# tychedelia/josefine

Hardware: NVIDIA H100
Metric: Raft-group ticks/sec @ 64Ki groups x 5 replicas (higher is better)
Workload: dtype u64

## Files before the change

josefine_b200/csrc/sym_fold.cuh:

```cuda
#pragma once
#include "raft_device.cuh"

namespace jr {
#ifdef JR_DEVICE_CODE

struct SymMail {
  uint32_t hb, hb_commit;
  uint32_t ae, ae_nb, ae_id[JR_MAX_AE_BLOCKS];
  uint32_t mk;
  uint32_t hbr, hbr_commit, hbr_has;
  uint32_t ar, ar_head;
};

constexpr uint32_t SYM_ROWS = 8;
#ifndef JR_SYM_LANES
#define JR_SYM_LANES 128
#endif
constexpr uint32_t SYM_LANES = JR_SYM_LANES;
constexpr uint32_t SYM_ENC_L = 5, SYM_ENC_F = 3;
constexpr uint32_t SYM_SMEM_UNITS = 2 * SYM_ROWS + SYM_ENC_L + SYM_ENC_F;
constexpr uint32_t SYM2_GROUPS = 64;
constexpr uint32_t SYM2_UNITS = SYM_SMEM_UNITS + 2 * 2 + 2 * 1;
constexpr uint32_t SYM2_ABORT = 1u << 8, SYM2_IDS = 1u << 9, SYM2_MODE = 1u << 10;

template <int R, bool SPLIT = false>
struct SymGroup {
  static constexpr uint32_t STRIDE = SPLIT ? SYM2_GROUPS : SYM_LANES;
  const Dev& d;
  const uint32_t g;
  const size_t plane;
  uint32_t L;
  uint32_t F0;
  uint64_t term, hbtime, now;
  uint32_t head, commit, idgen, maxkey, ckey, ph_self, mode_self, ph_f, mode_f;
  uint32_t fhead, fcommit, fmaxkey, fckey;
  uint32_t n_hb;
  uint64_t last_hb;
  uint32_t tbase;
  uint32_t flo;
  uint4* rows;
  uint4* enc;
  uint32_t lcnt, fcnt;
  uint32_t n_app;
  bool abort;
  bool share;

  __device__ __forceinline__ SymGroup(const Dev& dv, uint32_t g_) : d(dv), g(g_), plane((size_t)R * dv.Gp) {}
  __device__ __forceinline__ size_t rg(uint32_t r) const { return (size_t)r * d.Gp + g; }
  __device__ __forceinline__ size_t row(uint32_t r, uint32_t bid) const { return (size_t)(bid & d.capm) * plane + rg(r); }
  __device__ __forceinline__ bool in_window(uint32_t bid) const { return bid - tbase < d.cap; }
  __device__ __forceinline__ uint4& slot(uint32_t r, uint32_t bid) const { return rows[((r == L ? 0u : SYM_ROWS) + (bid % SYM_ROWS)) * STRIDE]; }
  __device__ __forceinline__ void cache_put(uint32_t r, uint32_t bid, uint32_t nx, uint64_t tk) const {
    slot(r, bid) = make_uint4(bid, nx, (uint32_t)tk, (uint32_t)(tk >> 32));
  }
  __device__ __forceinline__ void fetch(uint32_t r, uint32_t bid, uint32_t& next, uint64_t& tok) {
    if (!in_window(bid)) { next = ABSENT; tok = 0; return; }
    const uint4 e = slot(r, bid);
    if (e.x == bid) { next = e.y; tok = (uint64_t)e.z | ((uint64_t)e.w << 32); return; }
    next = __ldcg(d.cnext + row(r, bid));
    tok = __ldcg(d.ctok + row(r, bid));
    if (!SPLIT) cache_put(r, bid, next, tok);
  }
  __device__ __forceinline__ void fetch_sent(uint32_t bid, uint32_t mk_sent, uint32_t n_app, uint32_t& next, uint64_t& tok) {
    if (!SPLIT) { fetch(L, bid, next, tok); return; }
    if (!in_window(bid)) { next = ABSENT; tok = 0; return; }
    if (bid + SYM_ROWS > mk_sent + n_app) {
      const uint4 e = slot(L, bid);
      if (e.x == bid) { next = e.y; tok = (uint64_t)e.z | ((uint64_t)e.w << 32); return; }
    }
    next = __ldcg(d.cnext + row(L, bid));
    tok = __ldcg(d.ctok + row(L, bid));
  }
  __device__ __forceinline__ void cache_clear(uint32_t first = 0, uint32_t n = 2 * SYM_ROWS) const {
#pragma unroll
    for (uint32_t k = 0; k < 2 * SYM_ROWS; ++k)
      if (k >= first && k < first + n) rows[k * STRIDE] = make_uint4(ABSENT, ABSENT, 0u, 0u);
  }
  __device__ __forceinline__ void cache_fill(uint32_t r, uint32_t top) const {
    uint32_t nx[SYM_ROWS];
    uint64_t tk[SYM_ROWS];
#pragma unroll
    for (uint32_t j = 0; j < SYM_ROWS; ++j)
      if (j <= top && in_window(top - j)) {
        nx[j] = d.cnext[row(r, top - j)];
        tk[j] = d.ctok[row(r, top - j)];
      }
#pragma unroll
    for (uint32_t j = 0; j < SYM_ROWS; ++j)
      if (j <= top && in_window(top - j)) cache_put(r, top - j, nx[j], tk[j]);
  }
  __device__ __forceinline__ bool has(uint32_t r, uint32_t bid) {
    uint32_t n; uint64_t t;
    fetch(r, bid, n, t);
    return n != ABSENT;
  }
  __device__ __forceinline__ void fetch_f(uint32_t bid, uint32_t& next, uint64_t& tok) {
    if (in_window(bid) && bid < flo) { abort = true; next = ABSENT; tok = 0; return; }
    fetch(F0, bid, next, tok);
  }
  __device__ __forceinline__ bool has_f(uint32_t bid) {
    uint32_t n; uint64_t t;
    fetch_f(bid, n, t);
    return n != ABSENT;
  }

  __device__ __forceinline__ uint4& eq(uint32_t k) const { return enc[k * STRIDE]; }
  __device__ __forceinline__ FsmOut leader_out() const { return FsmOut{d.fs + rg(L), plane, d.F, g, L}; }
  __device__ __forceinline__ FsmOut followers_out() const {
    return FsmOut{d.fs + rg(F0), plane, d.F, g, F0, ((1u << R) - 1u) & ~(1u << L)};
  }
  __device__ __forceinline__ void enc_init_leader(uint2 leader_fc) const {
    eq(0) = make_uint4(leader_fc.x, leader_fc.y, leader_fc.y, 0u);
#pragma unroll
    for (uint32_t k = 1; k < SYM_ENC_L; ++k) eq(k) = make_uint4(0u, 0u, 0u, 0u);
  }
  __device__ __forceinline__ void enc_init_followers() const {
#pragma unroll
    for (uint32_t k = SYM_ENC_L; k < SYM_ENC_L + SYM_ENC_F; ++k) eq(k) = make_uint4(0u, 0u, 0u, 0u);
  }
  template <bool NOTIFY>
  __device__ __forceinline__ void emit_leader(uint32_t bid, uint32_t nxa, uint64_t tok) {
    if (!(d.flags & JR_F_CAPTURE_FSM)) return;
    if (lcnt >= d.Fr) { abort = true; return; }
    FsmEnc e;
    const uint4 q0 = eq(0);
    e.nrec = q0.x; e.seq = q0.y + lcnt; e.wseq = q0.z; e.pb2 = q0.w;
    ++lcnt;
    const bool window = NOTIFY || e.seq + 1u - e.wseq == FS_PATTERN_BITS;
    uint4 q1 = make_uint4(0u, 0u, 0u, 0u);
    if (window) q1 = eq(1);
    e.pb0 = (uint64_t)q1.x | ((uint64_t)q1.y << 32);
    e.pb1 = (uint64_t)q1.z | ((uint64_t)q1.w << 32);
    const uint4 qr = eq(NOTIFY ? 4 : 2), qs = eq(3);
    FsmRun& run = NOTIFY ? e.rn : e.ra;
    run.next_id = qr.x; run.count = qr.y;
    run.last = (uint64_t)qr.z | ((uint64_t)qr.w << 32);
    run.stride = NOTIFY ? ((uint64_t)qs.z | ((uint64_t)qs.w << 32)) : ((uint64_t)qs.x | ((uint64_t)qs.y << 32));
    fsm_enc_push<NOTIFY>(e, leader_out(), bid, nxa, tok);
    if (e.nrec != q0.x || e.wseq != q0.z || e.pb2 != q0.w) eq(0) = make_uint4(e.nrec, q0.y, e.wseq, e.pb2);
    if (window) eq(1) = make_uint4((uint32_t)e.pb0, (uint32_t)(e.pb0 >> 32), (uint32_t)e.pb1, (uint32_t)(e.pb1 >> 32));
    eq(NOTIFY ? 4 : 2) = make_uint4(run.next_id, run.count, (uint32_t)run.last, (uint32_t)(run.last >> 32));
    uint2* st = reinterpret_cast<uint2*>(&eq(3)) + (NOTIFY ? 1 : 0);
    *st = make_uint2((uint32_t)run.stride, (uint32_t)(run.stride >> 32));
  }
  __device__ __forceinline__ uint2 leader_end() {
    FsmEnc e;
    const uint4 q0 = eq(0), q1 = eq(1), q2 = eq(2), q3 = eq(3), q4 = eq(4);
    e.nrec = q0.x; e.seq = q0.y + lcnt; e.wseq = q0.z; e.pb2 = q0.w;
    e.pb0 = (uint64_t)q1.x | ((uint64_t)q1.y << 32);
    e.pb1 = (uint64_t)q1.z | ((uint64_t)q1.w << 32);
    e.ra = FsmRun{q2.x, q2.y, (uint64_t)q2.z | ((uint64_t)q2.w << 32), (uint64_t)q3.x | ((uint64_t)q3.y << 32)};
    e.rn = FsmRun{q4.x, q4.y, (uint64_t)q4.z | ((uint64_t)q4.w << 32), (uint64_t)q3.z | ((uint64_t)q3.w << 32)};
    return fsm_enc_end(e, leader_out());
  }
  __device__ __forceinline__ void emit_followers(uint32_t bid, uint32_t next, uint64_t tok) {
    if (!(d.flags & JR_F_CAPTURE_FSM)) return;
    if (fcnt >= d.Fr) { abort = true; return; }
    if (share) {
      FsmEnc e;
      const uint4 q0 = eq(SYM_ENC_L), q1 = eq(SYM_ENC_L + 1);
      const uint2 q2 = *reinterpret_cast<const uint2*>(&eq(SYM_ENC_L + 2));
      e.nrec = q0.x; e.seq = q0.y + fcnt; e.wseq = q0.z; e.pb2 = 0;
      e.pb0 = e.pb1 = 0;
      e.ra = FsmRun{q1.x, q1.y, (uint64_t)q1.z | ((uint64_t)q1.w << 32), (uint64_t)q2.x | ((uint64_t)q2.y << 32)};
      fsm_enc_push<false>(e, followers_out(), bid, next, tok);
      if (e.nrec != q0.x || e.wseq != q0.z) eq(SYM_ENC_L) = make_uint4(e.nrec, q0.y, e.wseq, 0u);
      eq(SYM_ENC_L + 1) = make_uint4(e.ra.next_id, e.ra.count, (uint32_t)e.ra.last, (uint32_t)(e.ra.last >> 32));
      *reinterpret_cast<uint2*>(&eq(SYM_ENC_L + 2)) = make_uint2((uint32_t)e.ra.stride, (uint32_t)(e.ra.stride >> 32));
    } else {
      const uint4 e = make_uint4(bid, next, (uint32_t)tok, (uint32_t)(tok >> 32));
#pragma unroll
      for (int r = 0; r < R; ++r)
        if ((uint32_t)r != L) d.fr[(size_t)fcnt * plane + rg(r)] = e;
    }
    ++fcnt;
  }
  __device__ __forceinline__ uint2 followers_end() {
    FsmEnc e;
    const uint4 q0 = eq(SYM_ENC_L), q1 = eq(SYM_ENC_L + 1), q2 = eq(SYM_ENC_L + 2);
    e.nrec = q0.x; e.seq = q0.y + fcnt; e.wseq = q0.z; e.pb2 = 0;
    e.pb0 = e.pb1 = 0;
    e.ra = FsmRun{q1.x, q1.y, (uint64_t)q1.z | ((uint64_t)q1.w << 32), (uint64_t)q2.x | ((uint64_t)q2.y << 32)};
    e.rn = FsmRun{0, 0, 0, 0};
    return fsm_enc_end(e, followers_out());
  }

  __device__ __forceinline__ uint32_t committed_index(uint32_t v_new, uint32_t n_new, uint32_t v_old) const {
    uint32_t v[R];
    v[0] = ph_self;
#pragma unroll
    for (int i = 1; i < R; ++i) v[i] = (uint32_t)i <= n_new ? v_new : v_old;
#pragma unroll
    for (int i = 0; i < R; ++i)
#pragma unroll
      for (int j = 0; j + 1 < R - i; ++j) {
        const uint32_t a = v[j], b = v[j + 1];
        v[j] = max(a, b);
        v[j + 1] = min(a, b);
      }
    return v[R / 2];
  }
  __device__ __forceinline__ void leader_commit(uint32_t v_new, uint32_t n_new, uint32_t v_old) {
    const uint32_t above = (ph_self > commit ? 1u : 0u) + (v_new > commit ? n_new : 0u) + (v_old > commit ? (uint32_t)(R - 1) - n_new : 0u);
    if (above < (uint32_t)(R / 2 + 1)) return;
    const uint32_t q = committed_index(v_new, n_new, v_old);
    if (q <= commit) return;
    if (!has(L, q)) { abort = true; return; }
    const uint32_t prev = commit;
    ckey = 1;
    commit = q;
    bool first = true;
    for (uint32_t b = max(prev, tbase); b <= q; ++b) {
      uint32_t nx; uint64_t tk;
      fetch(L, b, nx, tk);
      if (nx == ABSENT) continue;
      if (first) { first = false; continue; }
      emit_leader<false>(b, nx, tk);
    }
  }
  __device__ __forceinline__ void client_request(uint64_t tok) {
    const uint32_t bid = idgen++;
    if (!(bid > head) || !in_window(bid)) { abort = true; return; }
    d.cnext[row(L, bid)] = head;
    d.ctok[row(L, bid)] = tok;
    cache_put(L, bid, head, tok);
    if (bid > maxkey) maxkey = bid;
    head = bid;
    emit_leader<true>(bid, FSR_CLIENT, tok);
    mode_self = ph_self < head ? 1u : 0u;
    if (ph_self < head) ph_self = head;
    leader_commit(ph_f, R - 1, ph_f);
  }

  __device__ __forceinline__ void leader_tick(const SymMail& in, SymMail& out, uint64_t dense_tok, uint32_t n_synth,
                                              uint64_t step_index) {
    if (in.hbr && !in.hbr_has && in.hbr_commit > 0) { abort = true; return; }
    if (in.ar) {
      const uint32_t old = ph_f, v = in.ar_head;
      const bool inc = old < v;
      const uint32_t nw = inc ? v : old;
      for (uint32_t j = 1; j <= (uint32_t)(R - 1) && !abort; ++j) leader_commit(nw, j, old);
      ph_f = nw;
      mode_f = inc ? 1u : 0u;
      if (abort) return;
    }
    if (dense_tok) client_request(dense_tok);
    for (uint32_t i = 0; i < n_synth && !abort; ++i) client_request(synth_token(step_index, i, d.goff + g));
    if (abort) return;
    const uint64_t el = now >= hbtime ? now - hbtime : 0;
    if (el > (uint64_t)d.hb) {
      out.hb = 1;
      out.hb_commit = commit;
      hbtime = now;
    }
    out.ae = 1;
    out.mk = maxkey;
    if (!SPLIT) replicate(ph_f, mode_f, maxkey, out);
  }
  __device__ __forceinline__ void replicate(uint32_t phf, uint32_t modef, uint32_t mk, SymMail& out) {
    const uint32_t take = modef ? JR_MAX_AE_BLOCKS : 1u;
    uint32_t bid = max(phf, tbase), pulled = 0, nb = 0;
    while (pulled < 1 + take) {
      uint32_t nx = ABSENT; uint64_t tk = 0;
      while (bid <= mk) {
        fetch(L, bid, nx, tk);
        if (nx != ABSENT) break;
        ++bid;
      }
      if (bid > mk) break;
      if (pulled >= 1) out.ae_id[nb++] = bid;
      ++pulled;
      ++bid;
    }
    out.ae_nb = nb;
  }

  __device__ __forceinline__ void follower_heartbeat(const SymMail& in, SymMail& out) {
    ++n_hb;
    last_hb = now;
    const uint32_t c = in.hb_commit;
    const bool hasc = has_f(c);
    if (hasc && c > fcommit) {
      const uint32_t prev = fcommit;
      fckey = 1;
      fcommit = c;
      for (uint32_t b = max(prev, tbase); b < c; ++b) {
        uint32_t nx; uint64_t tk;
        fetch_f(b, nx, tk);
        if (nx != ABSENT) emit_followers(b, nx, tk);
      }
    }
    out.hbr = 1;
    out.hbr_commit = fcommit;
    out.hbr_has = hasc ? 1u : 0u;
  }
  __device__ __forceinline__ void follower_extend(uint32_t bid, uint32_t nx, uint64_t tk) {
    if (nx == ABSENT || !has_f(nx) || !in_window(bid)) { abort = true; return; }
#pragma unroll
    for (int r = 0; r < R; ++r)
      if ((uint32_t)r != L) {
        d.cnext[row(r, bid)] = nx;
        d.ctok[row(r, bid)] = tk;
      }
    cache_put(F0, bid, nx, tk);
    if (bid > fmaxkey) fmaxkey = bid;
    fhead = bid;
  }
  __device__ __forceinline__ void follower_tick(const SymMail& in, SymMail& out) {
    if (in.hb) follower_heartbeat(in, out);
    if (in.ae) {
      for (uint32_t k = 0; k < in.ae_nb && !abort; ++k) {
        const uint32_t bid = in.ae_id[k];
        uint32_t nx; uint64_t tk;
        fetch_sent(bid, in.mk, n_app, nx, tk);
        follower_extend(bid, nx, tk);
      }
      if (abort) return;
      if (in.ae_nb) {
        out.ar = 1;
        out.ar_head = fhead;
      }
    }
  }
  __device__ __forceinline__ void follower_tick_view(const SymMail& in, uint32_t phf, uint32_t modef, uint32_t mk, SymMail& out) {
    if (in.hb) follower_heartbeat(in, out);
    if (!in.ae || abort) return;
    const uint32_t take = modef ? JR_MAX_AE_BLOCKS : 1u;
    uint32_t bid = max(phf, tbase), pulled = 0, nb = 0;
    while (pulled < 1 + take) {
      uint32_t nx = ABSENT; uint64_t tk = 0;
      while (bid <= mk) {
        fetch_sent(bid, mk, n_app, nx, tk);
        if (nx != ABSENT) break;
        ++bid;
      }
      if (bid > mk) break;
      if (pulled >= 1) {
        follower_extend(bid, nx, tk);
        if (abort) return;
        ++nb;
      }
      ++pulled;
      ++bid;
    }
    if (nb) {
      out.ar = 1;
      out.ar_head = fhead;
    }
  }
};

template <int R, bool SPLIT>
__device__ __forceinline__ bool sym_enter(SymGroup<R, SPLIT>& s, SymMail& m, const StepParams& p, int prv) {
  const Dev& d = s.d;
  if (s.g >= d.G) return false;
  uint32_t L = R, nlead = 0;
  uint4 p2[R];
#pragma unroll
  for (int r = 0; r < R; ++r) {
    p2[r] = d.p2[s.rg(r)];
    const uint32_t meta = p2[r].w;
    if (((meta >> 8) & 255u) || ((meta >> 27) & 1u)) return false;
    if ((meta & 255u) == JR_ROLE_LEADER) { L = r; ++nlead; }
    else if ((meta & 255u) != JR_ROLE_FOLLOWER) return false;
    if ((meta >> 24) & 7u) return false;
  }
  if (nlead != 1) return false;
  s.L = L;
  s.F0 = L == 0 ? 1u : 0u;
  const uint4 l0 = d.p0[s.rg(L)];
  s.term = (uint64_t)l0.x | ((uint64_t)l0.y << 32);
  s.tbase = d.tb[s.g];
  uint4 pl = p2[0], pf = p2[0];
  const uint32_t f0i = L == 0 ? 1u : 0u;
#pragma unroll
  for (int r = 0; r < R; ++r) {
    if ((uint32_t)r == L) pl = p2[r];
    if ((uint32_t)r == f0i) pf = p2[r];
  }
  s.head = pl.x; s.commit = pl.y; s.idgen = pl.z;
  s.ckey = (pl.w >> 28) & 1u;
  s.maxkey = d.mk[s.rg(L)];
  if (!(s.idgen > s.head)) return false;
  const uint4 l3 = d.p3[s.rg(L)];
  s.hbtime = (uint64_t)l3.x | ((uint64_t)l3.y << 32);
  const uint32_t f0 = s.F0;
  s.fhead = pf.x; s.fcommit = pf.y; s.fckey = (pf.w >> 28) & 1u;
  s.fmaxkey = d.mk[s.rg(f0)];
  const uint64_t hbgap = ((uint64_t)d.hb / p.dt + 1) * p.dt;
#pragma unroll
  for (int r = 0; r < R; ++r) {
    if ((uint32_t)r == L) continue;
    const uint4 a = d.p0[s.rg(r)];
    if (((uint64_t)a.x | ((uint64_t)a.y << 32)) != s.term || a.z != L + 1 || a.w != L + 1) return false;
    if (p2[r].x != s.fhead || p2[r].y != s.fcommit || ((p2[r].w >> 28) & 1u) != s.fckey) return false;
    if (d.mk[s.rg(r)] != s.fmaxkey) return false;
  }
  if ((uint64_t)d.emin <= hbgap || s.hbtime > p.now) return false;
  uint32_t ph[R];
#pragma unroll
  for (int q = 0; q < (R + 3) / 4; ++q) {
    const uint4 v = d.pr[(size_t)q * s.plane + s.rg(L)];
    if (q * 4 + 0 < R) ph[q * 4 + 0] = v.x;
    if (q * 4 + 1 < R) ph[q * 4 + 1] = v.y;
    if (q * 4 + 2 < R) ph[q * 4 + 2] = v.z;
    if (q * 4 + 3 < R) ph[q * 4 + 3] = v.w;
  }
  const uint32_t prmask = (pl.w >> 16) & 255u;
  s.ph_self = 0; s.ph_f = 0;
#pragma unroll
  for (int r = 0; r < R; ++r) {
    if ((uint32_t)r == L) s.ph_self = ph[r];
    if ((uint32_t)r == f0) s.ph_f = ph[r];
  }
  s.mode_self = (prmask >> L) & 1u;
  s.mode_f = (prmask >> f0) & 1u;
#pragma unroll
  for (int r = 0; r < R; ++r)
    if ((uint32_t)r != L && (ph[r] != s.ph_f || ((prmask >> r) & 1u) != s.mode_f)) return false;
  constexpr uint32_t SYM_WINDOW = 16;
  const uint32_t top = min(s.maxkey, s.fmaxkey);
  const uint32_t lo_min = max(top > SYM_WINDOW - 1u ? top - (SYM_WINDOW - 1u) : 0u, s.tbase);
  if (top < s.tbase || s.ph_f < lo_min || s.fcommit < lo_min || s.commit < lo_min || s.fhead < lo_min || s.fmaxkey > s.maxkey) return false;
  const uint32_t lo = min(min(s.ph_f, s.fcommit), min(s.commit, s.fhead));
  s.flo = lo;
  const uint64_t grow = (uint64_t)p.n_ticks * (1u + p.n_synth) + 2u;
  if ((uint64_t)s.maxkey + grow >= (uint64_t)s.tbase + d.cap || (uint64_t)s.maxkey + grow >= FS_NOTIFY_BIT) return false;
  {
    constexpr uint32_t B = 4;
    bool same = true;
    for (uint32_t b0 = lo; b0 <= s.fmaxkey && same; b0 += B) {
      uint32_t n0[B];
      unsigned long long t0[B];
#pragma unroll
      for (uint32_t j = 0; j < B; ++j) {
        const uint32_t b = min(b0 + j, s.fmaxkey);
        n0[j] = d.cnext[s.row(f0, b)];
        t0[j] = d.ctok[s.row(f0, b)];
      }
#pragma unroll
      for (int r = 0; r < R; ++r) {
        if ((uint32_t)r == L || (uint32_t)r == f0) continue;
#pragma unroll
        for (uint32_t j = 0; j < B; ++j) {
          const uint32_t b = min(b0 + j, s.fmaxkey);
          const uint32_t n = d.cnext[s.row(r, b)];
          const unsigned long long t = d.ctok[s.row(r, b)];
          same = same && n == n0[j] && (n0[j] == ABSENT || t == t0[j]);
        }
      }
    }
    if (!same) return false;
  }
  m = SymMail{};
  if (p.phases & PH_DRAIN) {
  {
    const uint32_t cnt = d.oc[prv][s.rg(L)];
    uint32_t u = 0;
    auto unit = [&](uint32_t k) { return d.ob[prv][((size_t)k * R + L) * d.Gp + s.g]; };
    if (cnt > (uint32_t)(1 + JR_MAX_AE_BLOCKS + R)) return false;
    if (u < cnt) {
      const uint4 h = unit(u);
      if ((h.x & 15u) == JR_CMD_HEARTBEAT) {
        if ((h.x >> 16) != TO_PEERS || ((uint64_t)h.y | ((uint64_t)h.z << 32)) != s.term) return false;
        m.hb = 1; m.hb_commit = h.w;
        ++u;
      }
    }
    if (u < cnt) {
      uint32_t first = 0;
      for (int r = 0; r < R; ++r) {
        if ((uint32_t)r == L) continue;
        if (u >= cnt) return false;
        const uint4 h = unit(u);
        if ((h.x & 15u) != JR_CMD_APPEND_ENTRIES || (h.x >> 16) != (uint32_t)r + 1u ||
            ((uint64_t)h.y | ((uint64_t)h.z << 32)) != s.term) return false;
        const uint32_t nb = (h.x >> 8) & 255u, ref = (h.x >> 4) & 1u;
        if (!m.ae) {
          if (ref || nb > JR_MAX_AE_BLOCKS || h.w != u + 1 || u + 1 + nb > cnt) return false;
          m.ae = 1; m.ae_nb = nb; first = u + 1;
          for (uint32_t k = 0; k < nb; ++k) {
            const uint4 bu = unit(first + k);
            uint32_t nx; uint64_t tk;
            s.fetch(L, bu.x, nx, tk);
            if (nx != bu.y || tk != ((uint64_t)bu.z | ((uint64_t)bu.w << 32))) return false;
            m.ae_id[k] = bu.x;
          }
          u += 1 + nb;
        } else {
          if (!ref || nb != m.ae_nb || h.w != first) return false;
          ++u;
        }
      }
    }
    if (u != cnt) return false;
  }
  {
    const uint32_t cnt = d.oc[prv][s.rg(f0)];
    if (cnt > 2) return false;
    uint4 want[2] = {make_uint4(0, 0, 0, 0), make_uint4(0, 0, 0, 0)};
    for (uint32_t u = 0; u < cnt; ++u) want[u] = d.ob[prv][((size_t)u * R + f0) * d.Gp + s.g];
#pragma unroll
    for (int r = 0; r < R; ++r) {
      if ((uint32_t)r == L || (uint32_t)r == f0) continue;
      if (d.oc[prv][s.rg(r)] != cnt) return false;
      for (uint32_t u = 0; u < cnt; ++u) {
        const uint4 v = d.ob[prv][((size_t)u * R + r) * d.Gp + s.g];
        if (v.x != want[u].x || v.y != want[u].y || v.z != want[u].z || v.w != want[u].w) return false;
      }
    }
    uint32_t u = 0;
    if (u < cnt && (want[u].x & 15u) == JR_CMD_HEARTBEAT_RESPONSE) {
      if ((want[u].x >> 16) != L + 1) return false;
      m.hbr = 1; m.hbr_has = (want[u].x >> 4) & 1u; m.hbr_commit = want[u].w;
      ++u;
    }
    if (u < cnt && (want[u].x & 15u) == JR_CMD_APPEND_RESPONSE) {
      if ((want[u].x >> 16) != L + 1 || ((uint64_t)want[u].y | ((uint64_t)want[u].z << 32)) != s.term) return false;
      m.ar = 1; m.ar_head = want[u].w;
      ++u;
    }
    if (u != cnt) return false;
  }
  }
  uint64_t t_arr = 0;
  if (!m.hb) {
    const uint64_t due = s.hbtime + (uint64_t)d.hb + 1;
    t_arr = (due > p.now ? (due - p.now + p.dt - 1) / p.dt : 0) + 1;
  }
  const uint64_t checked = t_arr < p.n_ticks ? t_arr : p.n_ticks;
  if (checked) {
    const uint64_t t_last = p.now + (checked - 1) * p.dt;
#pragma unroll
    for (int r = 0; r < R; ++r) {
      if ((uint32_t)r == L) continue;
      const uint4 b = d.p1[s.rg(r)];
      const uint64_t etime = (uint64_t)b.x | ((uint64_t)b.y << 32);
      if (t_last >= etime && t_last - etime > (uint64_t)b.z) return false;
    }
  }
  return true;
}

template <int R, bool SPLIT>
__device__ __forceinline__ void sym_leave_leader(SymGroup<R, SPLIT>& s, const SymMail& last, int cur_last) {
  const Dev& d = s.d;
  const uint32_t L = s.L;
  {
    const size_t i = s.rg(L);
    uint32_t prmask = 0;
#pragma unroll
    for (int r = 0; r < R; ++r) prmask |= (((uint32_t)r == L ? s.mode_self : s.mode_f) & 1u) << r;
    const uint32_t keep = d.p2[i].w & ~((255u << 16) | (1u << 28));
    d.p2[i] = make_uint4(s.head, s.commit, s.idgen, keep | (prmask << 16) | (s.ckey << 28));
    d.p3[i] = make_uint4((uint32_t)s.hbtime, (uint32_t)(s.hbtime >> 32), 0u, 0u);
#pragma unroll
    for (int q = 0; q < (R + 3) / 4; ++q) {
      uint32_t v[4] = {0, 0, 0, 0};
#pragma unroll
      for (int k = 0; k < 4; ++k)
        if (q * 4 + k < R) v[k] = (uint32_t)(q * 4 + k) == L ? s.ph_self : s.ph_f;
      d.pr[(size_t)q * s.plane + i] = make_uint4(v[0], v[1], v[2], v[3]);
    }
    d.mk[i] = s.maxkey;
    uint32_t u = 0;
    auto put = [&](uint32_t k, uint4 v) { d.ob[cur_last][((size_t)k * R + L) * d.Gp + s.g] = v; };
    if (last.hb) put(u++, make_uint4(unit_hdr(JR_CMD_HEARTBEAT, 0, 0, TO_PEERS), (uint32_t)s.term, (uint32_t)(s.term >> 32), last.hb_commit));
    if (last.ae) {
      uint32_t first = 0;
      bool have = false;
#pragma unroll
      for (int r = 0; r < R; ++r) {
        if ((uint32_t)r == L) continue;
        if (!have) {
          first = u + 1;
          put(u, make_uint4(unit_hdr(JR_CMD_APPEND_ENTRIES, 0, last.ae_nb, r + 1), (uint32_t)s.term, (uint32_t)(s.term >> 32), first));
          for (uint32_t k = 0; k < last.ae_nb; ++k) {
            uint32_t nx; uint64_t tk;
            s.fetch(L, last.ae_id[k], nx, tk);
            put(first + k, make_uint4(last.ae_id[k], nx, (uint32_t)tk, (uint32_t)(tk >> 32)));
          }
          u += 1 + last.ae_nb;
          have = true;
        } else {
          put(u++, make_uint4(unit_hdr(JR_CMD_APPEND_ENTRIES, 1, last.ae_nb, r + 1), (uint32_t)s.term, (uint32_t)(s.term >> 32), first));
        }
      }
    }
    d.oc[cur_last][i] = u;
    if ((d.flags & JR_F_CAPTURE_FSM) && s.lcnt) d.fc[i] = s.leader_end();
  }
}

template <int R, bool SPLIT>
__device__ __forceinline__ void sym_leave_followers(SymGroup<R, SPLIT>& s, const SymMail& last, int cur_last) {
  const Dev& d = s.d;
  const uint32_t L = s.L;
  const bool shared_records = s.share;
#pragma unroll
  for (int r = 0; r < R; ++r) {
    if ((uint32_t)r == L) continue;
    const size_t i = s.rg(r);
    if (s.n_hb) {
      const uint4 b = d.p1[i];
      const uint32_t draws = b.w + s.n_hb;
      d.p1[i] = make_uint4((uint32_t)s.last_hb, (uint32_t)(s.last_hb >> 32),
                           election_timeout_draw(d.seed, d.goff + s.g, r + 1, draws - 1, d.emin, d.emax), draws);
    }
    const uint4 c = d.p2[i];
    d.p2[i] = make_uint4(s.fhead, s.fcommit, c.z, (c.w & ~(1u << 28)) | (s.fckey << 28));
    d.mk[i] = s.fmaxkey;
    uint32_t u = 0;
    if (last.hbr)
      d.ob[cur_last][((size_t)u++ * R + r) * d.Gp + s.g] =
          make_uint4(unit_hdr(JR_CMD_HEARTBEAT_RESPONSE, last.hbr_has, 0, L + 1), 0u, 0u, last.hbr_commit);
    if (last.ar)
      d.ob[cur_last][((size_t)u++ * R + r) * d.Gp + s.g] =
          make_uint4(unit_hdr(JR_CMD_APPEND_RESPONSE, 1, 0, L + 1), (uint32_t)s.term, (uint32_t)(s.term >> 32), last.ar_head);
    d.oc[cur_last][i] = u;
    if ((d.flags & JR_F_CAPTURE_FSM) && s.fcnt) {
      if (!shared_records) fsm_flush(d.fr + i, s.fcnt, d.Fr, FsmOut{d.fs + i, s.plane, d.F, s.g, (uint32_t)r}, d.fc + i);
      else if ((uint32_t)r == s.F0) d.fc[i] = s.followers_end();
      else d.fc[i] = make_uint2(0u, s.fcnt);
    }
  }
}

template <int R>
__global__ void __launch_bounds__(SYM_LANES, 512 / SYM_LANES) sym_kernel(const Dev d, const StepParams p, uint8_t* symdone) {
  const uint32_t g = blockIdx.x * blockDim.x + threadIdx.x;
  if (g >= d.Gp) return;
  SymGroup<R> s(d, g);
  SymMail a, b;
  s.abort = false;
  s.lcnt = s.fcnt = 0;
  s.n_hb = 0;
  s.last_hb = 0;
  s.share = false;
  s.n_app = 1u + p.n_synth;
  __shared__ uint4 lane_smem[SYM_SMEM_UNITS * SYM_LANES];
  s.rows = lane_smem + threadIdx.x;
  s.enc = lane_smem + 2 * SYM_ROWS * SYM_LANES + threadIdx.x;
  s.cache_clear();
  bool ok = sym_enter(s, a, p, 1 - p.cur);
  if (ok) {
    s.cache_fill(s.L, s.maxkey);
    s.cache_fill(s.F0, s.fmaxkey);
    s.share = (d.flags & JR_F_CAPTURE_FSM) != 0;
#pragma unroll
    for (int r = 0; r < R; ++r) {
      if ((uint32_t)r == s.L) continue;
      const uint2 c = d.fc[s.rg(r)];
      if (c.x | c.y) s.share = false;
    }
    s.enc_init_leader((d.flags & JR_F_CAPTURE_FSM) ? d.fc[s.rg(s.L)] : make_uint2(0u, 0u));
    s.enc_init_followers();
    const jr_proposal* props = p.proposals;
    s.now = p.now;
    for (uint32_t t = 0; t < p.n_ticks && !s.abort; ++t) {
      b = SymMail{};
      uint64_t tok = 0;
      if ((p.phases & PH_PROPOSE) && (props || p.tok_runs)) {
        uint4 pr;
        if (p.tok_runs) {
          const uint4 rn = __ldg(p.tok_runs + g);
          const uint64_t base = (uint64_t)rn.x | ((uint64_t)rn.y << 32);
          const uint64_t tk = base + (uint64_t)(p.tok_tick + t) * ((uint64_t)rn.z | ((uint64_t)rn.w << 32));
          pr = make_uint4((uint32_t)tk, (uint32_t)(tk >> 32), base ? __ldg(p.tok_route + g) : 0u, 0u);
        } else {
          pr = __ldg(reinterpret_cast<const uint4*>(props) + g);
          props += p.prop_stride;
        }
        if (pr.z == s.L + 1) tok = (uint64_t)pr.x | ((uint64_t)pr.y << 32);
        else if (pr.z != 0) s.abort = true;
      }
      if (s.abort) break;
      s.leader_tick(a, b, tok, (p.phases & PH_PROPOSE) ? p.n_synth : 0u, p.step_index + t);
      if (s.abort) break;
      s.follower_tick(a, b);
      a = b;
      s.now += p.dt;
    }
    ok = !s.abort;
    if (ok) {
      const int cur_last = p.cur ^ (int)((p.n_ticks - 1) & 1u);
      sym_leave_leader(s, a, cur_last);
      sym_leave_followers(s, a, cur_last);
    }
  }
  symdone[g] = ok ? 1 : 0;
}

#ifndef JR_SYM2_MINCTAS
#define JR_SYM2_MINCTAS 4
#endif
#ifndef JR_SYM2_ROLES
#define JR_SYM2_ROLES 3
#endif
template <int R>
__global__ void __launch_bounds__(2 * SYM2_GROUPS, JR_SYM2_MINCTAS) sym2_kernel(const Dev d, const StepParams p, uint8_t* symdone, uint8_t* symblk) {
  JR_DYN_SMEM(uint4, smem);
  auto pair_sync = [] { __syncthreads(); };
  constexpr uint32_t S = SYM2_GROUPS;
  const uint32_t w = threadIdx.x >> 5, lane = threadIdx.x & 31u;
  const bool lead = ((w ^ blockIdx.x) & 1u) == 0;
  const uint32_t gi = (w >> 1) * 32u + lane;
  const uint32_t g = blockIdx.x * S + gi;
  SymGroup<R, true> s(d, g);
  s.abort = false;
  s.lcnt = s.fcnt = 0;
  s.n_hb = 0;
  s.last_hb = 0;
  s.share = false;
  s.n_app = 1u + p.n_synth;
  s.rows = smem + gi;
  s.enc = smem + 2 * SYM_ROWS * S + gi;
  uint4* mail = smem + SYM_SMEM_UNITS * S + gi;
  s.cache_clear(lead ? 0u : SYM_ROWS, SYM_ROWS);
  const uint32_t blk = g / GROUPS_PER_CTA;
  if (lead && lane == 0 && g < d.Gp) symblk[blk] = 1;
  pair_sync();
  SymMail a;
  bool dead = !sym_enter(s, a, p, 1 - p.cur);
  pair_sync();
  if (!dead) {
    if (lead) {
      s.cache_fill(s.L, s.maxkey);
      s.enc_init_leader((d.flags & JR_F_CAPTURE_FSM) ? d.fc[s.rg(s.L)] : make_uint2(0u, 0u));
      mail[2 * S] = make_uint4(a.hb | (a.ae << 1) | (a.ae_nb << 4) | SYM2_IDS, a.hb_commit, s.maxkey, a.ae_id[0]);
      mail[3 * S] = make_uint4(a.ae_id[1], a.ae_id[2], a.ae_id[3], a.ae_id[4]);
    } else {
      s.cache_fill(s.F0, s.fmaxkey);
      s.enc_init_followers();
      s.share = (d.flags & JR_F_CAPTURE_FSM) != 0;
#pragma unroll
      for (int r = 0; r < R; ++r) {
        if ((uint32_t)r == s.L) continue;
        const uint2 c = d.fc[s.rg(r)];
        if (c.x | c.y) s.share = false;
      }
      mail[5 * S] = make_uint4(a.hbr | (a.hbr_has << 1) | (a.ar << 2), a.hbr_commit, a.ar_head, 0u);
    }
  }
  pair_sync();
  const jr_proposal* props = p.proposals;
  s.now = p.now;
  uint32_t cur = 0;
  for (uint32_t t = 0; t < p.n_ticks; ++t) {
    if (lead && (JR_SYM2_ROLES & 1)) {
      if (!dead) {
        const uint4 c = mail[(4 + (1 - cur)) * S];
        if (c.x & SYM2_ABORT) dead = true;
        else {
          SymMail in{}, out{};
          in.hbr = c.x & 1u; in.hbr_has = (c.x >> 1) & 1u; in.ar = (c.x >> 2) & 1u;
          in.hbr_commit = c.y; in.ar_head = c.z;
          uint64_t tok = 0;
          if ((p.phases & PH_PROPOSE) && (props || p.tok_runs)) {
            uint4 pr;
            if (p.tok_runs) {
              const uint4 rn = __ldg(p.tok_runs + g);
              const uint64_t base = (uint64_t)rn.x | ((uint64_t)rn.y << 32);
              const uint64_t tk = base + (uint64_t)(p.tok_tick + t) * ((uint64_t)rn.z | ((uint64_t)rn.w << 32));
              pr = make_uint4((uint32_t)tk, (uint32_t)(tk >> 32), base ? __ldg(p.tok_route + g) : 0u, 0u);
            } else {
              pr = __ldg(reinterpret_cast<const uint4*>(props + (size_t)t * p.prop_stride) + g);
            }
            if (pr.z == s.L + 1) tok = (uint64_t)pr.x | ((uint64_t)pr.y << 32);
            else if (pr.z != 0) s.abort = true;
          }
          if (!s.abort) s.leader_tick(in, out, tok, (p.phases & PH_PROPOSE) ? p.n_synth : 0u, p.step_index + t);
          if (s.abort) dead = true;
          else {
            mail[(2 * cur) * S] = make_uint4(out.hb | (out.ae << 1) | (s.mode_f ? SYM2_MODE : 0u), s.commit, s.maxkey, s.ph_f);
          }
        }
      }
      if (dead) mail[(2 * cur) * S] = make_uint4(SYM2_ABORT, 0u, 0u, 0u);
    } else if (!lead && (JR_SYM2_ROLES & 2)) {
      if (!dead) {
        const uint4 ma = mail[(2 * (1 - cur)) * S];
        if (ma.x & SYM2_ABORT) dead = true;
        else {
          SymMail in{}, out{};
          in.hb = ma.x & 1u; in.ae = (ma.x >> 1) & 1u;
          in.hb_commit = ma.y; in.mk = ma.z;
          if (ma.x & SYM2_IDS) {
            const uint4 mb = mail[(2 * (1 - cur) + 1) * S];
            in.ae_nb = (ma.x >> 4) & 15u;
            in.ae_id[0] = ma.w; in.ae_id[1] = mb.x; in.ae_id[2] = mb.y; in.ae_id[3] = mb.z; in.ae_id[4] = mb.w;
            s.follower_tick(in, out);
          } else {
            s.follower_tick_view(in, ma.w, (ma.x & SYM2_MODE) ? 1u : 0u, ma.z, out);
          }
          if (s.abort) dead = true;
          else mail[(4 + cur) * S] = make_uint4(out.hbr | (out.hbr_has << 1) | (out.ar << 2), out.hbr_commit, out.ar_head, 0u);
        }
      }
      if (dead) mail[(4 + cur) * S] = make_uint4(SYM2_ABORT, 0u, 0u, 0u);
    }
    s.now += p.dt;
    pair_sync();
    cur ^= 1u;
  }
  const uint32_t lastb = cur ^ 1u;
  const uint4 la = mail[(2 * lastb) * S], lc = mail[(4 + lastb) * S];
  const bool ok = !dead && !((la.x | lc.x) & SYM2_ABORT);
  if (ok) {
    const int cur_last = p.cur ^ (int)((p.n_ticks - 1) & 1u);
    SymMail last{};
    if (lead) {
      last.hb = la.x & 1u; last.ae = (la.x >> 1) & 1u;
      last.hb_commit = la.y;
      if (last.ae) s.replicate(s.ph_f, s.mode_f, s.maxkey, last);
      sym_leave_leader(s, last, cur_last);
    } else {
      last.hbr = lc.x & 1u; last.hbr_has = (lc.x >> 1) & 1u; last.ar = (lc.x >> 2) & 1u;
      last.hbr_commit = lc.y; last.ar_head = lc.z;
      sym_leave_followers(s, last, cur_last);
    }
  }
  if (p.trunc) {
    pair_sync();
    if (ok && !lead) {
      const uint32_t lo = min(s.fcommit, la.y);
      const uint32_t floor = lo > p.trunc_margin ? lo - p.trunc_margin : 0u;
      if (floor > s.tbase) {
        for (uint32_t b = s.tbase; b < floor && b - s.tbase < d.cap; ++b)
#pragma unroll
          for (int r = 0; r < R; ++r) d.cnext[s.row(r, b)] = ABSENT;
        d.tb[g] = floor;
      }
    }
  }
  if (lead && g < d.Gp) {
    symdone[g] = ok ? 1 : 0;
    if (!ok) {
      symblk[blk] = 0;
      if (g < d.G) *(volatile uint32_t*)d.hunf = p.epoch;
    }
  }
}

__global__ void sym_blocks_kernel(const uint8_t* symdone, uint8_t* symblk, uint32_t n_blocks) {
  const uint32_t b = blockIdx.x * blockDim.x + threadIdx.x;
  if (b >= n_blocks) return;
  const uint4* v = reinterpret_cast<const uint4*>(symdone + (size_t)b * GROUPS_PER_CTA);
  const uint4 x = v[0], y = v[1];
  const uint32_t all = 0x01010101u;
  symblk[b] = (x.x == all && x.y == all && x.z == all && x.w == all && y.x == all && y.y == all && y.z == all && y.w == all) ? 1 : 0;
}

#endif
}
```

Before: 10.48 billion.

## Add fast-path run extension in FSM encoders and profiling phase hooks

Adds a run_extend fast path to the leader and follower FSM encoders. When a new record just continues the current strided run, the code updates the run state in shared memory and skips the full FsmEnc decode, push and re-encode. It tracks window ends (lwend/fwend) so the slow path still runs at pattern-window boundaries. It also replaces dynamic ae_id array indexing with unrolled select loops so the array can stay in registers, and adds JR_PROFILE-gated phase timing hooks that compile to nothing by default. The fast path risks subtle divergence from the full encoder's run semantics.

```diff
diff --git a/josefine_b200/csrc/sym_fold.cuh b/josefine_b200/csrc/sym_fold.cuh
--- a/josefine_b200/csrc/sym_fold.cuh
+++ b/josefine_b200/csrc/sym_fold.cuh
@@ -10,6 +10,18 @@
   uint32_t mk;
   uint32_t hbr, hbr_commit, hbr_has;
   uint32_t ar, ar_head;
+  __device__ __forceinline__ uint32_t id(uint32_t k) const {
+    uint32_t v = ae_id[0];
+#pragma unroll
+    for (uint32_t j = 1; j < JR_MAX_AE_BLOCKS; ++j)
+      if (k == j) v = ae_id[j];
+    return v;
+  }
+  __device__ __forceinline__ void set_id(uint32_t k, uint32_t v) {
+#pragma unroll
+    for (uint32_t j = 0; j < JR_MAX_AE_BLOCKS; ++j)
+      if (k == j) ae_id[j] = v;
+  }
 };
 
 constexpr uint32_t SYM_ROWS = 8;
@@ -22,6 +34,19 @@
 constexpr uint32_t SYM2_GROUPS = 64;
 constexpr uint32_t SYM2_UNITS = SYM_SMEM_UNITS + 2 * 2 + 2 * 1;
 constexpr uint32_t SYM2_ABORT = 1u << 8, SYM2_IDS = 1u << 9, SYM2_MODE = 1u << 10;
+enum : uint32_t {
+  SP_MAIL_IN = 0,
+  SP_AR = 1,
+  SP_CLIENT = 2,
+  SP_ENC_NOTIFY = 3,
+  SP_ENC_APPLY = 4,
+  SP_MAIL_OUT = 5,
+  SP_BARRIER = 6,
+  SP_HB = 7,
+  SP_SCAN = 8,
+  SP_EXTEND = 9,
+  SP_ENTER = 10, SP_FILL = 11, SP_LEAVE = 12, SP_TRUNC = 13,
+};
 
 template <int R, bool SPLIT = false>
 struct SymGroup {
@@ -41,11 +66,30 @@
   uint4* rows;
   uint4* enc;
   uint32_t lcnt, fcnt;
+  uint32_t lwend, fwend;
   uint32_t n_app;
   bool abort;
   bool share;
-
-  __device__ __forceinline__ SymGroup(const Dev& dv, uint32_t g_) : d(dv), g(g_), plane((size_t)R * dv.Gp) {}
+#ifdef JR_PROFILE
+  long long pt;
+  uint32_t prole, pslot;
+  __device__ __forceinline__ uint32_t phase(uint32_t slot) {
+    const uint32_t o = pslot;
+    if constexpr (SPLIT) {
+      JR_PROF_ADD(prole, o, pt);
+      pslot = slot;
+    }
+    return o;
+  }
+#else
+  __device__ __forceinline__ uint32_t phase(uint32_t) const { return 0; }
+#endif
+
+  __device__ __forceinline__ SymGroup(const Dev& dv, uint32_t g_) : d(dv), g(g_), plane((size_t)R * dv.Gp) {
+#ifdef JR_PROFILE
+    pt = 0; prole = JR_ROLE_CANDIDATE; pslot = 0;
+#endif
+  }
   __device__ __forceinline__ size_t rg(uint32_t r) const { return (size_t)r * d.Gp + g; }
   __device__ __forceinline__ size_t row(uint32_t r, uint32_t bid) const { return (size_t)(bid & d.capm) * plane + rg(r); }
   __device__ __forceinline__ bool in_window(uint32_t bid) const { return bid - tbase < d.cap; }
@@ -109,19 +153,48 @@
   __device__ __forceinline__ FsmOut followers_out() const {
     return FsmOut{d.fs + rg(F0), plane, d.F, g, F0, ((1u << R) - 1u) & ~(1u << L)};
   }
-  __device__ __forceinline__ void enc_init_leader(uint2 leader_fc) const {
+  __device__ __forceinline__ void enc_init_leader(uint2 leader_fc) {
     eq(0) = make_uint4(leader_fc.x, leader_fc.y, leader_fc.y, 0u);
 #pragma unroll
     for (uint32_t k = 1; k < SYM_ENC_L; ++k) eq(k) = make_uint4(0u, 0u, 0u, 0u);
-  }
-  __device__ __forceinline__ void enc_init_followers() const {
+    lwend = FS_PATTERN_BITS;
+  }
+  __device__ __forceinline__ void enc_init_followers() {
 #pragma unroll
     for (uint32_t k = SYM_ENC_L; k < SYM_ENC_L + SYM_ENC_F; ++k) eq(k) = make_uint4(0u, 0u, 0u, 0u);
+    fwend = FS_PATTERN_BITS;
+  }
+  template <bool NOTIFY>
+  __device__ __forceinline__ bool run_extend(uint4& q, uint2& qs, uint32_t bid, uint32_t nxa, uint64_t tok) const {
+    const uint4 r = q;
+    if (!r.y || bid != r.x || r.y >= FS_MAX_RUN || nxa != (NOTIFY ? FSR_CLIENT : bid - 1u)) return false;
+    const uint2 st = qs;
+    const uint64_t step = tok - ((uint64_t)r.z | ((uint64_t)r.w << 32));
+    if (r.y == 1u) {
+      if (st.x != (NOTIFY ? FSR_CLIENT : bid - 2u)) return false;
+      qs = make_uint2((uint32_t)step, (uint32_t)(step >> 32));
+    } else if (step != ((uint64_t)st.x | ((uint64_t)st.y << 32))) {
+      return false;
+    }
+    q = make_uint4(bid + 1u, r.y + 1u, (uint32_t)tok, (uint32_t)(tok >> 32));
+    return true;
   }
   template <bool NOTIFY>
   __device__ __forceinline__ void emit_leader(uint32_t bid, uint32_t nxa, uint64_t tok) {
     if (!(d.flags & JR_F_CAPTURE_FSM)) return;
     if (lcnt >= d.Fr) { abort = true; return; }
+    const uint32_t outer = phase(NOTIFY ? SP_ENC_NOTIFY : SP_ENC_APPLY);
+    if (lcnt + 1u != lwend &&
+        run_extend<NOTIFY>(eq(NOTIFY ? 4 : 2), reinterpret_cast<uint2*>(&eq(3))[NOTIFY ? 1 : 0], bid, nxa, tok)) {
+      if (NOTIFY) {
+        const uint32_t b = lcnt + FS_PATTERN_BITS - lwend;
+        uint32_t* w = b < 128u ? reinterpret_cast<uint32_t*>(&eq(1)) + (b >> 5) : &eq(0).w;
+        *w |= 1u << (b & 31u);
+      }
+      ++lcnt;
+      phase(outer);
+      return;
+    }
     FsmEnc e;
     const uint4 q0 = eq(0);
     e.nrec = q0.x; e.seq = q0.y + lcnt; e.wseq = q0.z; e.pb2 = q0.w;
@@ -142,6 +215,8 @@
     eq(NOTIFY ? 4 : 2) = make_uint4(run.next_id, run.count, (uint32_t)run.last, (uint32_t)(run.last >> 32));
     uint2* st = reinterpret_cast<uint2*>(&eq(3)) + (NOTIFY ? 1 : 0);
     *st = make_uint2((uint32_t)run.stride, (uint32_t)(run.stride >> 32));
+    lwend = e.wseq - q0.y + FS_PATTERN_BITS;
+    phase(outer);
   }
   __device__ __forceinline__ uint2 leader_end() {
     FsmEnc e;
@@ -156,7 +231,10 @@
   __device__ __forceinline__ void emit_followers(uint32_t bid, uint32_t next, uint64_t tok) {
     if (!(d.flags & JR_F_CAPTURE_FSM)) return;
     if (fcnt >= d.Fr) { abort = true; return; }
-    if (share) {
+    const uint32_t outer = phase(SP_ENC_APPLY);
+    if (share && fcnt + 1u != fwend &&
+        run_extend<false>(eq(SYM_ENC_L + 1), *reinterpret_cast<uint2*>(&eq(SYM_ENC_L + 2)), bid, next, tok)) {
+    } else if (share) {
       FsmEnc e;
       const uint4 q0 = eq(SYM_ENC_L), q1 = eq(SYM_ENC_L + 1);
       const uint2 q2 = *reinterpret_cast<const uint2*>(&eq(SYM_ENC_L + 2));
@@ -167,6 +245,7 @@
       if (e.nrec != q0.x || e.wseq != q0.z) eq(SYM_ENC_L) = make_uint4(e.nrec, q0.y, e.wseq, 0u);
       eq(SYM_ENC_L + 1) = make_uint4(e.ra.next_id, e.ra.count, (uint32_t)e.ra.last, (uint32_t)(e.ra.last >> 32));
       *reinterpret_cast<uint2*>(&eq(SYM_ENC_L + 2)) = make_uint2((uint32_t)e.ra.stride, (uint32_t)(e.ra.stride >> 32));
+      fwend = e.wseq - q0.y + FS_PATTERN_BITS;
     } else {
       const uint4 e = make_uint4(bid, next, (uint32_t)tok, (uint32_t)(tok >> 32));
 #pragma unroll
@@ -174,6 +253,7 @@
         if ((uint32_t)r != L) d.fr[(size_t)fcnt * plane + rg(r)] = e;
     }
     ++fcnt;
+    phase(outer);
   }
   __device__ __forceinline__ uint2 followers_end() {
     FsmEnc e;
@@ -236,6 +316,7 @@
                                               uint64_t step_index) {
     if (in.hbr && !in.hbr_has && in.hbr_commit > 0) { abort = true; return; }
     if (in.ar) {
+      phase(SP_AR);
       const uint32_t old = ph_f, v = in.ar_head;
       const bool inc = old < v;
       const uint32_t nw = inc ? v : old;
@@ -244,9 +325,11 @@
       mode_f = inc ? 1u : 0u;
       if (abort) return;
     }
+    phase(SP_CLIENT);
     if (dense_tok) client_request(dense_tok);
     for (uint32_t i = 0; i < n_synth && !abort; ++i) client_request(synth_token(step_index, i, d.goff + g));
     if (abort) return;
+    phase(SP_MAIL_OUT);
     const uint64_t el = now >= hbtime ? now - hbtime : 0;
     if (el > (uint64_t)d.hb) {
       out.hb = 1;
@@ -268,7 +351,7 @@
         ++bid;
       }
       if (bid > mk) break;
-      if (pulled >= 1) out.ae_id[nb++] = bid;
+      if (pulled >= 1) out.set_id(nb++, bid);
       ++pulled;
       ++bid;
     }
@@ -276,6 +359,7 @@
   }
 
   __device__ __forceinline__ void follower_heartbeat(const SymMail& in, SymMail& out) {
+    phase(SP_HB);
     ++n_hb;
     last_hb = now;
     const uint32_t c = in.hb_commit;
@@ -295,6 +379,7 @@
     out.hbr_has = hasc ? 1u : 0u;
   }
   __device__ __forceinline__ void follower_extend(uint32_t bid, uint32_t nx, uint64_t tk) {
+    const uint32_t outer = phase(SP_EXTEND);
     if (nx == ABSENT || !has_f(nx) || !in_window(bid)) { abort = true; return; }
 #pragma unroll
     for (int r = 0; r < R; ++r)
@@ -305,12 +390,14 @@
     cache_put(F0, bid, nx, tk);
     if (bid > fmaxkey) fmaxkey = bid;
     fhead = bid;
+    phase(outer);
   }
   __device__ __forceinline__ void follower_tick(const SymMail& in, SymMail& out) {
     if (in.hb) follower_heartbeat(in, out);
     if (in.ae) {
+      phase(SP_SCAN);
       for (uint32_t k = 0; k < in.ae_nb && !abort; ++k) {
-        const uint32_t bid = in.ae_id[k];
+        const uint32_t bid = in.id(k);
         uint32_t nx; uint64_t tk;
         fetch_sent(bid, in.mk, n_app, nx, tk);
         follower_extend(bid, nx, tk);
@@ -325,6 +412,7 @@
   __device__ __forceinline__ void follower_tick_view(const SymMail& in, uint32_t phf, uint32_t modef, uint32_t mk, SymMail& out) {
     if (in.hb) follower_heartbeat(in, out);
     if (!in.ae || abort) return;
+    phase(SP_SCAN);
     const uint32_t take = modef ? JR_MAX_AE_BLOCKS : 1u;
     uint32_t bid = max(phf, tbase), pulled = 0, nb = 0;
     while (pulled < 1 + take) {
@@ -484,7 +572,7 @@
             uint32_t nx; uint64_t tk;
             s.fetch(L, bu.x, nx, tk);
             if (nx != bu.y || tk != ((uint64_t)bu.z | ((uint64_t)bu.w << 32))) return false;
-            m.ae_id[k] = bu.x;
+            m.set_id(k, bu.x);
           }
           u += 1 + nb;
         } else {
@@ -576,9 +664,10 @@
           first = u + 1;
           put(u, make_uint4(unit_hdr(JR_CMD_APPEND_ENTRIES, 0, last.ae_nb, r + 1), (uint32_t)s.term, (uint32_t)(s.term >> 32), first));
           for (uint32_t k = 0; k < last.ae_nb; ++k) {
+            const uint32_t bid = last.id(k);
             uint32_t nx; uint64_t tk;
-            s.fetch(L, last.ae_id[k], nx, tk);
-            put(first + k, make_uint4(last.ae_id[k], nx, (uint32_t)tk, (uint32_t)(tk >> 32)));
+            s.fetch(L, bid, nx, tk);
+            put(first + k, make_uint4(bid, nx, (uint32_t)tk, (uint32_t)(tk >> 32)));
           }
           u += 1 + last.ae_nb;
           have = true;
@@ -716,6 +805,12 @@
   s.rows = smem + gi;
   s.enc = smem + 2 * SYM_ROWS * S + gi;
   uint4* mail = smem + SYM_SMEM_UNITS * S + gi;
+#ifdef JR_PROFILE
+  for (uint32_t i = threadIdx.x; i < 8 * 3 * 16 * 2; i += blockDim.x) jr_prof_smem()[i] = 0;
+  s.prole = lead ? JR_ROLE_LEADER : JR_ROLE_FOLLOWER;
+  s.pslot = SP_ENTER;
+  s.pt = clock64();
+#endif
   s.cache_clear(lead ? 0u : SYM_ROWS, SYM_ROWS);
   const uint32_t blk = g / GROUPS_PER_CTA;
   if (lead && lane == 0 && g < d.Gp) symblk[blk] = 1;
@@ -723,6 +818,7 @@
   SymMail a;
   bool dead = !sym_enter(s, a, p, 1 - p.cur);
   pair_sync();
+  s.phase(SP_FILL);
   if (!dead) {
     if (lead) {
       s.cache_fill(s.L, s.maxkey);
@@ -747,6 +843,7 @@
   s.now = p.now;
   uint32_t cur = 0;
   for (uint32_t t = 0; t < p.n_ticks; ++t) {
+    s.phase(SP_MAIL_IN);
     if (lead && (JR_SYM2_ROLES & 1)) {
       if (!dead) {
         const uint4 c = mail[(4 + (1 - cur)) * S];
@@ -793,6 +890,7 @@
           } else {
             s.follower_tick_view(in, ma.w, (ma.x & SYM2_MODE) ? 1u : 0u, ma.z, out);
           }
+          s.phase(SP_MAIL_OUT);
           if (s.abort) dead = true;
           else mail[(4 + cur) * S] = make_uint4(out.hbr | (out.hbr_has << 1) | (out.ar << 2), out.hbr_commit, out.ar_head, 0u);
         }
@@ -800,9 +898,11 @@
       if (dead) mail[(4 + cur) * S] = make_uint4(SYM2_ABORT, 0u, 0u, 0u);
     }
     s.now += p.dt;
+    s.phase(SP_BARRIER);
     pair_sync();
     cur ^= 1u;
   }
+  s.phase(SP_LEAVE);
   const uint32_t lastb = cur ^ 1u;
   const uint4 la = mail[(2 * lastb) * S], lc = mail[(4 + lastb) * S];
   const bool ok = !dead && !((la.x | lc.x) & SYM2_ABORT);
@@ -820,6 +920,7 @@
       sym_leave_followers(s, last, cur_last);
     }
   }
+  s.phase(SP_TRUNC);
   if (p.trunc) {
     pair_sync();
     if (ok && !lead) {
@@ -840,6 +941,15 @@
       if (g < d.G) *(volatile uint32_t*)d.hunf = p.epoch;
     }
   }
+#ifdef JR_PROFILE
+  s.phase(SP_TRUNC);
+  __syncthreads();
+  if (d.prof)
+    for (uint32_t i = threadIdx.x; i < 4 * 3 * 16 * 2; i += blockDim.x) {
+      const unsigned long long v = jr_prof_smem()[i];
+      if (v) atomicAdd(d.prof + (i % (3 * 16 * 2)), v);
+    }
+#endif
 }
 
 __global__ void sym_blocks_kernel(const uint8_t* symdone, uint8_t* symblk, uint32_t n_blocks) {
```

Result: faster. 11.18 billion, median of 6 (+6.7%).
